# giech/usrp_nfc

Hardware: AMD Instinct MI355X
Metric: IQ Msamples/s -> decoded bits (2 Msps stream) (higher is better)
Workload: dtype f32 envelope / f64 window sums / u8 symbols; 1 GPU; configs[1]: Miller-only decode, synthetic IQ @2 Msps; input_kind=fc32 IQ, 8 B/sample (envelope computed in the kernel), samples_per_gpu=100000000, parallelism=time-chunk x1, edges_per_gpu=6627699, symbols_reader=3971547, symbols_tag=0, packets=101186, boundary_redos=0, exchange=none, stepping=sync, in_flight=1

## Files before the change

### usrp_nfc_amd/csrc/decode.hip.h

```cpp
#pragma once
#include <hip/hip_runtime.h>
#include <stdint.h>

#include "../../include/nfc_amd.h"
#include "scan.hip.h"

namespace nfc {

struct DecTables {
    const uint4 *mil_map;
    const uint2 *man_map;
    const uint16_t *mil_step;
    const uint16_t *man_step;
    int32_t nd;
    int32_t reader, tag;
    const uint2 *qmil_map;
    const uint16_t *qmil_step;
    uint32_t q_rep[2];
    uint32_t canon[4];
    int32_t q_ok;
};
__device__ __forceinline__ uint32_t byte_of(const uint32_t *w, uint32_t i) { return (w[i >> 2] >> (8u * (i & 3u))) & 0xFFu; }

struct DecCarry {
    int32_t mil_state, man_state;
    int32_t pkt_started[2];
    uint32_t pending[2];
};

constexpr int DEC_ITEMS = 16;
#ifndef NFC_DEC_GROUPS
#define NFC_DEC_GROUPS 2
#endif
constexpr int DEC_GROUPS = NFC_DEC_GROUPS;
constexpr int DEC_PER_THREAD = DEC_ITEMS * DEC_GROUPS;
constexpr int DEC_TILE = SCAN_BLOCK * DEC_PER_THREAD;
constexpr int DEC_LDS_ROWS = 512;
inline size_t dec_num_tiles(size_t n) { return (n + DEC_TILE - 1) / DEC_TILE; }

enum DecLdsUser { DEC_LDS_SPEC = 0, DEC_LDS_REDUCE = 1, DEC_LDS_APPLY = 2 };
inline size_t dec_table_bytes(DecLdsUser k, const DecTables &T) {
    const size_t rows = 4 * (size_t)T.nd, nr = T.reader ? 1 : 0, nt = T.tag ? 1 : 0;
    if (rows > (size_t)DEC_LDS_ROWS) return 0;
    switch (k) {
    case DEC_LDS_SPEC: return (nr + nt) * (rows * 16 + (rows + 1) * 8);
    case DEC_LDS_REDUCE: return nr * rows * 16 + nt * rows * 8;
    default: return nr * rows * 32 + nt * rows * 16;
    }
}

__device__ __forceinline__ void load_codes(const uint16_t *ecode, size_t base, size_t n, uint32_t (&c)[8]) {
    if (base + DEC_ITEMS <= n) {
        const uint4 a = *(const uint4 *)(ecode + base), b = *(const uint4 *)(ecode + base + 8);
        c[0] = a.x; c[1] = a.y; c[2] = a.z; c[3] = a.w;
        c[4] = b.x; c[5] = b.y; c[6] = b.z; c[7] = b.w;
    } else {
#pragma unroll
        for (int k = 0; k < 8; k++) {
            const size_t i = base + 2 * k;
            c[k] = (i < n ? (uint32_t)ecode[i] : 0u) | (i + 1 < n ? (uint32_t)ecode[i + 1] << 16 : 0u);
        }
    }
}
__device__ __forceinline__ void load_bytes16(const uint8_t *p, size_t base, size_t n, uint32_t fill, uint32_t (&w)[4]) {
    if (base + 16 <= n) {
        const uint4 a = *(const uint4 *)(p + base);
        w[0] = a.x; w[1] = a.y; w[2] = a.z; w[3] = a.w;
    } else {
#pragma unroll
        for (int k = 0; k < 4; k++) {
            uint32_t v = 0;
#pragma unroll
            for (int q = 0; q < 4; q++) {
                const size_t i = base + 4 * k + q;
                v |= (i < n ? (uint32_t)p[i] : fill) << (8 * q);
            }
            w[k] = v;
        }
    }
}

constexpr uint32_t PM_STOP = 0u, PM_START = 1u, PM_ID = 2u;
constexpr uint32_t FA_DB = 4u, FA_DC = 8u;
struct FrameAgg {
    uint32_t cnt[2];
    uint32_t nb[2], nc[2];
    uint32_t fl[2];
};
struct FrameAggOp {
    using T = FrameAgg;
    static __host__ __device__ __forceinline__ T identity() { return T{{0u, 0u}, {0u, 0u}, {0u, 0u}, {PM_ID, PM_ID}}; }
    static __device__ __forceinline__ T op(const T &a, const T &b) {
        T r;
#pragma unroll
        for (int t = 0; t < 2; t++) {
            const uint32_t ma = a.fl[t] & 3u, mb = b.fl[t] & 3u;
            const bool into_stopped = ma == PM_STOP;
            r.cnt[t] = a.cnt[t] + b.cnt[t];
            r.nb[t] = a.nb[t] + b.nb[t] - (into_stopped ? (b.fl[t] >> 2) & 1u : 0u);
            r.nc[t] = a.nc[t] + b.nc[t] - (into_stopped ? (b.fl[t] >> 3) & 1u : 0u);
            r.fl[t] = (mb == PM_ID ? ma : mb) | ((ma == PM_ID ? b.fl[t] : a.fl[t]) & (FA_DB | FA_DC));
        }
        return r;
// ... 242 lines not shown
            const uint32_t code = (c[g][k >> 1] >> (16 * (k & 1))) & 0xFFFFu;
            const uint32_t li = code & 0x3FFFu, route = code >> 14;
            uint32_t w = 0;
            if (route == 2u && T.reader) {
                const uint32_t e = mil[li * 16u + (st & 15u)];
                w = e >> 8;
                st = (st & ~15u) | (e & 15u);
            } else if (route == 1u && T.tag) {
                const uint32_t e = man[li * 8u + ((st >> 4) & 7u)];
                const uint32_t m = e >> 8;
                w = (m & 3u) ? ((m & 0xFCu) | 3u) : 0u;
                st = (st & 15u) | ((e & 15u) << 4);
            }
            ow[k >> 2] |= w << (8 * (k & 3));
        }
        const size_t gb = base + (size_t)DEC_ITEMS * g;
        if (gb < n) *(uint4 *)(outw + gb) = make_uint4(ow[0], ow[1], ow[2], ow[3]);
        mine = FramePkOp::op(mine, FramePkOp::pack(frame_agg_of(ow)));
    }
    TP_MARK();
    FramePk total_fa;
    *(uint4 *)(thread_aggs + tid) = make_uint4(mine.a[0], mine.a[1], mine.b[0], mine.b[1]);
    (void)block_exclusive<FramePkOp>(mine, lds2, total_fa);
    if (threadIdx.x == 0) frame_aggs[blockIdx.x] = FramePkOp::unpack(total_fa);
    TP_DONE(2);
}

constexpr int FW_WORDS = DEC_TILE * 2 / 32 + 4;
constexpr uint32_t ST_CLOSES = 512 * DEC_GROUPS;
struct TileStage {
    uint32_t *bits[2];
    uint32_t *close_bit[2];
    uint64_t *close_idx[2];
    uint32_t *drop_bit[2];
    FrameAgg *own;
    const uint32_t *epos;
    uint64_t g0;
    const uint64_t *idx64;
};
__device__ __forceinline__ void bitcopy_or(uint32_t *dst, uint32_t dst_bit, const uint32_t *src, uint32_t src_bit, uint32_t nbits, uint32_t cap_bits) {
    if (!nbits) return;
    const uint32_t w0 = dst_bit >> 5, nw = ((dst_bit & 31u) + nbits + 31u) >> 5, capw = (cap_bits + 31u) >> 5;
    for (uint32_t j = threadIdx.x; j < nw; j += blockDim.x) {
        if (w0 + j >= capw) break;
        const uint32_t lo = max(dst_bit, (w0 + j) << 5), hi = min(dst_bit + nbits, (w0 + j + 1u) << 5);
        const uint32_t sb = src_bit + (lo - dst_bit), k = sb & 31u;
        const uint32_t a = src[sb >> 5], b = k ? src[(sb >> 5) + 1u] : 0u;
        uint32_t v = (a >> k) | (k ? b << (32u - k) : 0u);
        const uint32_t cnt = hi - lo;
        if (cnt < 32u) v &= (1u << cnt) - 1u;
        v <<= (lo & 31u);
        if (v) atomicOr(dst + w0 + j, v);
    }
}

struct QMaps {
    uint32_t mil[2];
    uint32_t man[2];
};
struct ComposeQ {
    using T = QMaps;
    static __host__ __device__ __forceinline__ T identity() { return T{{0x03020100u, 0x07060504u}, {0x03020100u, 0x07060504u}}; }
    static __device__ __forceinline__ T op(const T &a, const T &b) {
        return T{{__builtin_amdgcn_perm(b.mil[1], b.mil[0], a.mil[0]), __builtin_amdgcn_perm(b.mil[1], b.mil[0], a.mil[1])},
                 {__builtin_amdgcn_perm(b.man[1], b.man[0], a.man[0]), __builtin_amdgcn_perm(b.man[1], b.man[0], a.man[1])}};
    }
    static __device__ __forceinline__ uint32_t step(const T &m, uint32_t st) {
        const uint32_t a = __builtin_amdgcn_perm(m.mil[1], m.mil[0], st & 7u) & 15u;
        const uint32_t b = __builtin_amdgcn_perm(m.man[1], m.man[0], (st >> 4) & 7u) & 15u;
        return a | (b << 4);
    }
};
struct DecSpec {
    QMaps map;
    uint32_t s_in;
    uint32_t needs;
    uint32_t pad[2];
};
static_assert(sizeof(DecSpec) == 32, "two 16-byte loads");
__device__ __forceinline__ bool map8_constant(const uint32_t (&m)[2]) { return m[0] == m[1] && m[0] == (m[0] & 0xFFu) * 0x01010101u; }
constexpr int DEC_RUNIN_MAX = 8;
static_assert(DEC_GROUPS >= 1 && DEC_GROUPS <= 2, "NFC_DEC_GROUPS: a thread's packed bits are accumulated in 64 bits (32 slots per group)");
static_assert(DEC_RUNIN_MAX * SCAN_BLOCK <= DEC_TILE, "the longest run-in fits inside the tile before");
template <bool LDS, int DECS>
__global__ __launch_bounds__(SCAN_BLOCK) void k_dec_spec(const uint16_t *ecode, size_t n, const uint32_t *n_dev, DecTables T, uint32_t state0, int runin_per_thread,
                                                        uint8_t *outw, FrameAgg *frame_aggs, DecSpec *spec, ZeroJob Z, TileStage S) {
    constexpr bool RD = (DECS & 1) != 0, TG = (DECS & 2) != 0;
    zero_words(Z);
    if (n_dev) n = min(n, (size_t)*n_dev);
    if ((size_t)blockIdx.x * DEC_TILE >= n) return;
    TP_DECL();
    extern __shared__ __attribute__((aligned(16))) unsigned char s_dec_tab[];
    const int trows = LDS ? 4 * T.nd : 0;
    uint16_t *const s_mil = (uint16_t *)s_dec_tab, *const s_man = s_mil + (RD ? trows * 8 : 0);
    uint2 *const s_milmap = (uint2 *)(s_man + (TG ? trows * 8 : 0)), *const s_manmap = s_milmap + (LDS && RD ? trows + 1 : 0);
    __shared__ QMaps lds[SCAN_WAVES];
    __shared__ FramePk lds2[SCAN_WAVES];
    __shared__ uint32_t s_needs;
    __shared__ uint32_t s_bits[2][FW_WORDS];
    __shared__ uint32_t s_drop[2];
    for (int i = threadIdx.x; i < 2 * FW_WORDS; i += SCAN_BLOCK) (&s_bits[0][0])[i] = 0u;
    if (threadIdx.x < 2) s_drop[threadIdx.x] = 0xFFFFFFFFu;
    const uint32_t ident = 4u * (uint32_t)T.nd;
    if (LDS) {
        const int rows = 4 * T.nd;
        for (int i = threadIdx.x; i <= rows; i += SCAN_BLOCK) {
            if (RD) s_milmap[i] = T.qmil_map[i];
            if (TG) s_manmap[i] = T.man_map[i];
        }
        for (int i = threadIdx.x; i < rows; i += SCAN_BLOCK) {
            if (RD) ((uint4 *)s_mil)[i] = ((const uint4 *)T.qmil_step)[i];
            if (TG) ((uint4 *)s_man)[i] = ((const uint4 *)T.man_step)[i];
        }
    }
    if (threadIdx.x == 0) s_needs = 0u;
    const size_t tid = (size_t)blockIdx.x * SCAN_BLOCK + threadIdx.x;
    const size_t base = tid * DEC_PER_THREAD;
    uint32_t c[DEC_GROUPS][8];
#pragma unroll
    for (int g = 0; g < DEC_GROUPS; g++) load_codes(ecode, base + DEC_ITEMS * g, n, c[g]);
    uint32_t rc[DEC_RUNIN_MAX / 2];
    const bool have_runin = blockIdx.x > 0;
    {
        const size_t r0 = (size_t)blockIdx.x * DEC_TILE - (size_t)runin_per_thread * SCAN_BLOCK + (size_t)threadIdx.x * runin_per_thread;
#pragma unroll
        for (int k = 0; k < DEC_RUNIN_MAX / 2; k++) rc[k] = (have_runin && 2 * k < runin_per_thread) ? *(const uint32_t *)(ecode + r0 + 2 * k) : 0u;
    }
    __syncthreads();
    TP_MARK();
    auto mil_row = [&](uint32_t code) __attribute__((always_inline)) -> uint2 {
        const uint32_t idx = (code >> 14) == 2u ? (code & 0x3FFFu) : ident;
        return LDS ? s_milmap[idx] : T.qmil_map[idx];
    };
    auto man_row = [&](uint32_t code) __attribute__((always_inline)) -> uint2 {
        const uint32_t idx = (code >> 14) == 1u ? (code & 0x3FFFu) : ident;
        return LDS ? s_manmap[idx] : T.man_map[idx];
    };
    auto then = [](const uint2 &a, const uint2 &b) __attribute__((always_inline)) -> uint2 {
        return make_uint2(__builtin_amdgcn_perm(b.y, b.x, a.x), __builtin_amdgcn_perm(b.y, b.x, a.y));
    };
    auto routes_of = [](uint32_t pair) __attribute__((always_inline)) -> uint32_t {
        const uint32_t r0 = (pair >> 14) & 3u, r1 = pair >> 30;
        return ((r0 == 2u || r1 == 2u) ? 1u : 0u) | ((r0 == 1u || r1 == 1u) ? 2u : 0u);
    };
    auto compose4 = [&](uint2 &am, uint2 &an, uint32_t w0, uint32_t w1) __attribute__((always_inline)) {
        const uint32_t c0 = w0 & 0xFFFFu, c1 = w0 >> 16, c2 = w1 & 0xFFFFu, c3 = w1 >> 16;
        if (RD) am = then(am, then(then(mil_row(c0), mil_row(c1)), then(mil_row(c2), mil_row(c3))));
        if (TG) an = then(an, then(then(man_row(c0), man_row(c1)), then(man_row(c2), man_row(c3))));
    };
    const QMaps idm = ComposeQ::identity();
    QMaps runin = idm;
    if (have_runin) {
        uint2 am = make_uint2(idm.mil[0], idm.mil[1]), an = make_uint2(idm.man[0], idm.man[1]);
#pragma unroll
        for (int k = 0; k < DEC_RUNIN_MAX / 2; k += 2)
            if (2 * k < runin_per_thread) compose4(am, an, rc[k], rc[k + 1]);
        const QMaps ra{{am.x, am.y}, {an.x, an.y}};
        (void)block_exclusive<ComposeQ>(ra, lds, runin);
    }
    uint32_t seen = 0u;
    uint2 am = make_uint2(idm.mil[0], idm.mil[1]), an = make_uint2(idm.man[0], idm.man[1]);
#ifndef NFC_DEC_CHAIN
#define NFC_DEC_CHAIN 8
#endif
    constexpr int CHAIN = NFC_DEC_CHAIN;
    static_assert(CHAIN == 16 || CHAIN == 8 || CHAIN == 4, "NFC_DEC_CHAIN");
    constexpr int NCH = DEC_PER_THREAD / CHAIN;
    uint2 pm[NCH], pn[NCH];
#pragma unroll
    for (int g = 0; g < DEC_GROUPS; g++) {
#pragma unroll
        for (int k = 0; k < 8; k += 2) {
            if (k % (CHAIN / 2) == 0) {
                pm[(16 * g + 2 * k) / CHAIN] = am;
                pn[(16 * g + 2 * k) / CHAIN] = an;
            }
            compose4(am, an, c[g][k], c[g][k + 1]);
            seen |= routes_of(c[g][k]) | routes_of(c[g][k + 1]);
        }
    }
    if (!RD) seen &= ~1u;
    if (!TG) seen &= ~2u;
    const QMaps agg{{am.x, am.y}, {an.x, an.y}};
    TP_MARK();
    QMaps total;
    const QMaps excl = block_exclusive<ComposeQ>(agg, lds, total);
    const QMaps upto = ComposeQ::op(runin, excl);
    const uint32_t dep = ((seen & 1u) && !map8_constant(upto.mil) ? 1u : 0u) | ((seen & 2u) && !map8_constant(upto.man) ? 2u : 0u);
    if (blockIdx.x > 0 && dep) atomicOr(&s_needs, dep);
    uint32_t st[NCH];
#pragma unroll
    for (int j = 0; j < NCH; j++) st[j] = ComposeQ::step(ComposeQ::op(upto, QMaps{{pm[j].x, pm[j].y}, {pn[j].x, pn[j].y}}), state0);
    TP_MARK();
    const uint16_t *mil = LDS ? s_mil : T.qmil_step;
    const uint16_t *man = LDS ? s_man : T.man_step;
    uint32_t ow[DEC_GROUPS][4];
#pragma unroll
    for (int g = 0; g < DEC_GROUPS; g++) ow[g][0] = ow[g][1] = ow[g][2] = ow[g][3] = 0u;
#pragma unroll
    for (int e = 0; e < CHAIN; e++) {
#pragma unroll
        for (int j = 0; j < NCH; j++) {
            const int g = (j * CHAIN) / DEC_ITEMS, k = (j * CHAIN) % DEC_ITEMS + e;
            const uint32_t code = (c[g][k >> 1] >> (16 * (k & 1))) & 0xFFFFu;
            const uint32_t li = code & 0x3FFFu, route = code >> 14;
            uint32_t w = 0;
            if (route == 2u && RD) {
                const uint32_t en = mil[li * 8u + (st[j] & 7u)];
                w = en >> 8;
                st[j] = (st[j] & ~15u) | (en & 15u);
            } else if (route == 1u && TG) {
                const uint32_t en = man[li * 8u + ((st[j] >> 4) & 7u)];
                const uint32_t m = en >> 8;
                w = (m & 3u) ? ((m & 0xFCu) | 3u) : 0u;
                st[j] = (st[j] & 15u) | ((en & 15u) << 4);
            }
            ow[g][k >> 2] |= w << (8 * (k & 3));
        }
    }
    FramePk mine = FramePkOp::identity();
#pragma unroll
    for (int g = 0; g < DEC_GROUPS; g++) {
        const size_t gb = base + (size_t)DEC_ITEMS * g;
        if (gb < n) *(uint4 *)(outw + gb) = make_uint4(ow[g][0], ow[g][1], ow[g][2], ow[g][3]);
        mine = FramePkOp::op(mine, FramePkOp::pack(frame_agg_of<DECS>(ow[g])));
    }
    TP_MARK();
    FramePk total_fa;
    const FramePk in_tile = block_exclusive<FramePkOp>(mine, lds2, total_fa);
    {
        FrameAgg before = FramePkOp::unpack(in_tile);
        uint64_t acc[2] = {0ull, 0ull};
        uint32_t cnt[2] = {0u, 0u};
        const uint32_t bo0[2] = {before.nb[0], before.nb[1]};
#pragma unroll
        for (int g = 0; g < DEC_GROUPS; g++) {
            if (ow[g][0] | ow[g][1] | ow[g][2] | ow[g][3]) {
                const SlotMasks m = slot_masks<DECS>(ow[g]);
                const uint32_t low = symbol_low_bits(ow[g]);
#pragma unroll
                for (int t = 0; t < 2; t++) {
                    if (!(t ? RD : TG) || !m.V[t]) continue;
                    const uint32_t started = pm_apply(before.fl[t], 1u);
                    const uint32_t bef = started_before(m, t, started);
                    const uint32_t appended = m.V[t] & ~m.ST[t] & (bef | ~m.SA[t]);
                    uint32_t cl = m.ST[t] & bef;
                    const uint32_t bo = bo0[t] + cnt[t];
                    const uint32_t nonid = m.ST[t] | m.SA[t];
                    if ((before.fl[t] & 3u) == PM_ID && nonid) {
                        const uint32_t first = nonid & (0u - nonid);
                        if (first & m.SA[t]) s_drop[t] = bo + (uint32_t)__popc(appended & (first - 1u));
                    }
                    acc[t] |= (uint64_t)compress32(low, appended) << cnt[t];
                    cnt[t] += (uint32_t)__popc(appended);
                    if (cl) {
                        const uint32_t co = before.nc[t], closes = cl;
                        while (cl) {
                            const uint32_t lowb = cl & (0u - cl);
                            const int k = (__ffs((int)cl) - 1) >> 1;
                            cl ^= lowb;
                            const uint32_t j = co + (uint32_t)__popc(closes & (lowb - 1u));
                            if (j < ST_CLOSES) {
                                const size_t e = base + (size_t)DEC_ITEMS * g + k;
                                S.close_bit[t][(size_t)blockIdx.x * ST_CLOSES + j] = bo + (uint32_t)__popc(appended & (lowb - 1u));
                                S.close_idx[t][(size_t)blockIdx.x * ST_CLOSES + j] = S.idx64 ? S.idx64[e] : S.g0 + (uint64_t)S.epos[e];
                            } else {
                                atomicOr(&s_needs, 4u);
                            }
                        }
                    }
                }
                if (g + 1 < DEC_GROUPS) before = FrameAggOp::op(before, frame_agg_of<DECS>(ow[g]));
            }
        }
#pragma unroll
        for (int t = 0; t < 2; t++) {
            if (!cnt[t]) continue;
            const uint32_t w = bo0[t] >> 5, sh = bo0[t] & 31u;
            const uint64_t lo = acc[t] << sh;
            const uint32_t hi = sh ? (uint32_t)(acc[t] >> (64u - sh)) : 0u;
            if (w + 2 < (uint32_t)FW_WORDS) {
                if ((uint32_t)lo) atomicOr(&s_bits[t][w], (uint32_t)lo);
                if ((uint32_t)(lo >> 32)) atomicOr(&s_bits[t][w + 1], (uint32_t)(lo >> 32));
                if (hi) atomicOr(&s_bits[t][w + 2], hi);
            }
        }
    }
    __syncthreads();
    const FrameAgg tile_fa = FramePkOp::unpack(total_fa);
#pragma unroll
    for (int t = 0; t < 2; t++) {
        if (!(t ? RD : TG)) continue;
        const uint32_t nw = min((uint32_t)FW_WORDS, (tile_fa.nb[t] + 31u) / 32u + 1u);
        for (uint32_t j = threadIdx.x; j < nw; j += SCAN_BLOCK) S.bits[t][(size_t)blockIdx.x * FW_WORDS + j] = s_bits[t][j];
    }
    if (threadIdx.x == 0) {
        frame_aggs[blockIdx.x] = tile_fa;
        S.own[blockIdx.x] = tile_fa;
        if (TG) S.drop_bit[0][blockIdx.x] = s_drop[0];
        if (RD) S.drop_bit[1][blockIdx.x] = s_drop[1];
// ... 439 lines not shown
```

### usrp_nfc_amd/csrc/decoder_tables.h

```cpp
#pragma once
#include <cmath>
#include <cstdint>
#include <vector>

namespace nfc {

enum : int { E_NONE = 0, E_TOO_SHORT = 2, E_TOO_LONG = 3, E_ENCODING = 4, E_INTERNAL = 5, E_WRONG_DUR = 6 };
constexpr double kFull = 9.44;
constexpr double kZero = 3.00;
constexpr double kHalf = kFull / 2;
constexpr double kZeroRem = kFull - kZero;
constexpr double kOneRem = kHalf - kZero;
constexpr double kOneHalf = kFull + kHalf;

enum : int { MS_BEGIN = 0, MS_ZS0 = 1, MS_OS0 = 2, MS_OS1 = 3 };
constexpr int kMillerStates = 16;
constexpr int kManchStates = 8;

struct Step {
    int next;
    int nout;
    int out[2];
};

// ... 141 lines not shown
                tm |= (uint32_t)(st.next & 15) << (4 * s);
                t.manch_out[((size_t)c * nd + d) * kManchStates + s] = pack_out(st);
            }
            t.manch_map[c * nd + d] = tm;
        }
    }
    return t;
}

struct MillerQuotient {
    bool ok = false;
    int classes = 0;
    uint8_t q_of[16], rep[8], canon[16];
    std::vector<uint64_t> map;
    std::vector<uint16_t> step;
};
inline MillerQuotient miller_quotient(const DecoderTables &t) {
    MillerQuotient q;
    const size_t rows = t.miller_map.size();
    int cls[16] = {0};
    for (;;) {
        int ncls[16], nid = 0;
        std::vector<std::vector<int>> sigs;
        for (int s = 0; s < 16; s++) {
            std::vector<int> sig{cls[s]};
            for (size_t r = 0; r < rows; r++) {
                sig.push_back(t.miller_out[r * 16 + s]);
                sig.push_back(cls[(t.miller_map[r] >> (4 * s)) & 15]);
            }
            int id = -1;
            for (int k = 0; k < nid; k++)
                if (sigs[k] == sig) id = k;
            if (id < 0) {
                id = nid++;
                sigs.push_back(sig);
            }
            ncls[s] = id;
        }
        bool same = true;
        for (int s = 0; s < 16; s++) same = same && ncls[s] == cls[s];
        for (int s = 0; s < 16; s++) cls[s] = ncls[s];
        if (same) break;
    }
    bool reach[16] = {false};
    reach[0] = true;
    for (bool grew = true; grew;) {
        grew = false;
        for (int s = 0; s < 16; s++)
            if (reach[s])
                for (size_t r = 0; r < rows; r++) {
                    const int nx = (int)((t.miller_map[r] >> (4 * s)) & 15);
                    if (!reach[nx]) reach[nx] = grew = true;
                }
    }
    int qid[16];
    for (int k = 0; k < 16; k++) qid[k] = -1;
    for (int s = 0; s < 16; s++)
        if (reach[s] && qid[cls[s]] < 0) {
            if (q.classes == 8) return q;
            q.rep[q.classes] = (uint8_t)s;
            qid[cls[s]] = q.classes++;
        }
    for (int s = 0; s < 16; s++) {
        q.q_of[s] = qid[cls[s]] >= 0 ? (uint8_t)qid[cls[s]] : (uint8_t)0xFF;
        q.canon[s] = qid[cls[s]] >= 0 ? q.rep[qid[cls[s]]] : (uint8_t)s;
    }
    for (int k = q.classes; k < 8; k++) q.rep[k] = q.rep[0];
    q.map.assign(rows, 0);
    q.step.assign(rows * 8, 0);
    for (size_t r = 0; r < rows; r++) {
        uint64_t m = 0;
        for (int k = 0; k < 8; k++) {
            const int s = q.rep[k < q.classes ? k : 0];
            const int nx = q.q_of[(t.miller_map[r] >> (4 * s)) & 15];
            m |= (uint64_t)nx << (8 * k);
            q.step[r * 8 + k] = (uint16_t)(nx | (t.miller_out[r * 16 + s] << 8));
        }
        q.map[r] = m;
    }
    q.ok = true;
    return q;
}

}
```

### usrp_nfc_amd/csrc/host_context.h

```cpp
#pragma once


namespace {

std::string g_create_error;

}

enum : int {
    TOT_RUNS = 0,
    TOT_EDGES = 8,
    TOT_DECMAP = 16,
    TOT_SPEC = 40,
    TOT_PKT0 = 72,
    TOT_PKT1 = 80,
    TOT_LAST2 = 88,
    TOT_NSYM = 96,
    TOT_CERT = 104,
    TOT_FRAME = 128,
    TOT_BYTES = 160
};

static_assert(sizeof(CertSummary) <= TOT_FRAME - TOT_CERT, "the verdict summary fits its slot of the totals");
struct DevState {
// ... 41 lines not shown
    if (const char *e = getenv("NFC_OWN_PREFIX_MAX")) s.own_prefix_max = strtoul(e, nullptr, 10);
    if (const char *e = getenv("NFC_WG_LONE")) {
        int a = 4, b = 64;
        if (sscanf(e, "%d,%d", &a, &b) >= 1) s.wg_lone = std::make_pair(a, b);
    }
    if (const char *e = getenv("NFC_WG_ROWBAL")) {
        std::array<double, 3> f{0.0, 1.0, 1.0};
        if (sscanf(e, "%lf,%lf,%lf", &f[0], &f[1], &f[2]) >= 2 && f[0] > 0.5 && f[0] < 1.5 && f[1] > 0.5 && f[1] < 1.5 && f[2] > 0.5 && f[2] < 1.5)
            s.rowbal_f = f;
        else s.wg_rowbal = atoi(e);
    }
    if (const char *e = getenv("NFC_RING")) {
        if (strcmp(e, "global") == 0) s.ring_global = true;
        else if (strcmp(e, "lds") == 0) s.ring_global = false;
    }
#endif
    return s;
}
}

struct nfc_ctx {
    nfc_params P;
    const KindKernels *kk = nullptr;
    int L, mx, Lpad, wpb, twords;
    double factor;
    double hi_plus, lo_a, lo_b, hi_a, hi_b;
    int bands_ok, fast_ok, nfold, wave_slots, lds_per_slot;
    int C_min;
    uint32_t ring_carried = 0;
    bool dec_spec = true, dec_spec_now = false;
    int dec_runin = 2, spec_off_left = 0, spec_fail_streak = 0;
    size_t dec_lds[3] = {0, 0, 0};
    bool bits_packed = false, sym_lazy = false, sym_own = false;
    FrameOut sym_P;
    uint32_t sym_n = 0, sym_tiles = 0;
    uint32_t decode_respeculated = 0;
    int lean = 1, lean_rounds = 0, lean_slots = 0;
    int n_cus = 1;
    double rowbal_f[5][3] = {{1, 1, 1}, {1, 1, 1}, {1.02, 1, 1}, {1.045, 1.004, 1}, {1.036, 1.015, 0.990}};
    bool rowbal_set = false;
    bool wg_rowbal = true;
    int wg = 1, wg_ok = 0, wg_nr = 4, wg_slots = 0, wg_slots_ahead = 0, wg_rounds = 0;
    int fine_left = 0, fine_adapt = 1, fine_mult = 4;
    size_t wg_lds = 0, wg_lds_base = 0, wg_lds_bulk_max = 0;
    bool wg_bulk = true;
    int wg_lone_max = 4, wg_lone_div = 64;
    int wg_rerun_lone = 1;
    int wg_ex_ok = 0, wg_ex_max = 0;
    size_t wg_ex_lds = 0;
    float lean_gfac = 1.3f, lean_gmin = 9.765625e-4f;
    int gring_ok = 0, gring_force = 0, wave_slots_g = 0;
    uint32_t own_prefix_max = OWN_PREFIX_MAX_TILES;
    int use_small = 1;
    double expect_ms = 0.3;
    bool spin_wait = true;
    uint64_t selmask;
    float eps;
    float i16_scale;
    size_t in_bytes_per_sample;
    hipStream_t st = nullptr;
    Stream own_st;
    Stream st_a;
    Event ev[8];
    DevBuf d_gring;
    bool state_dirty = false, dirty_fill_ring = false;
    float dirty_fill = 0.f;
    Carry dirty_carry;
    EdgeCarry dirty_ecarry;
    DecCarry dirty_dcarry;
    bool cert_pending = false;
    CertLaunch cert;
    bool fill_pending = false, fill_can_ride = false, fill_front = false;
    FillRider fill;
    uint32_t dbg_fill_rode = 0, dbg_fill_refront = 0;
    bool dbg_bad_launch = false, dbg_redo_submitted = false, dbg_no_submit_ahead = false, dbg_any = false, dbg_clk = false, dbg_trace = false;
    std::string dbg_clk_path;
    uint32_t batch_seq = 0;
    int timing = 0;
    Event kev[2 * 6];
    int n_kev = 0;
    std::string err;
    LaunchError launch_err;

    DevBuf d_mil_map, d_man_map, d_mil_out, d_man_out, d_qmil_map, d_qmil_step;
    uint8_t mil_q_of[16], mil_canon[16];
    DecTables T;

    DevBuf d_state, d_ring[NRING];
    PinBuf hs_pin{hipHostMallocMapped | hipHostMallocCoherent};
    DevState *hs = nullptr;
    void *hs_dev = nullptr;
    PinBuf h_stage;
    PinBuf h_pk_stage;
    PinBuf h_edge_stage;
    std::vector<uint64_t> edge_lut;
    PinBuf h_cflags;
    int ring_cur = 0;
    DevBuf d_neg_alt[NSUB - 1], d_pos_alt[NSUB - 1];
    uint32_t alt_free = (1u << (NSUB - 1)) - 1u;
    PinBuf hs_a[NSUB];
    Event ev_a[NSUB], ev_b[NSUB];
    Event kev_sub[NSUB][2];
    struct Submitted {
        const void *d_in = nullptr;
        uint32_t n = 0, seq = 0, nch = 0, chunk = 0;
        uint64_t g0 = 0;
        int slot = 0, planes = -1, ring_in = 0, timing = 0;
        uint32_t allocs = 0;
        bool fast = false, b_enqueued = false, timed = false, spec = false;
    } sub[NSUB];
    int sub_count = 0;
    uint32_t slot_next = 0;
    bool low_valid = false;
    size_t lean_lds_per_cu = 0;
    size_t ahead_lds_per_cu = 0;
    uint32_t stamp_b = 0;
    bool in_wait = false;
    uint32_t dbg_fast_waits = 0;
    uint32_t stats_redo_submitted = 0;
    Carry h_carry;
    EdgeCarry h_ecarry;
    DecCarry h_dcarry;
    uint64_t nseen = 0;

    DevBuf d_certinfo;
    DevBuf d_in, d_neg, d_pos, d_ringout[2], d_touched[2], d_info[2], d_ringin, d_meta, d_ver, d_cflags, d_list;
    DevBuf d_ecode, d_epos, d_eidx;
    bool edges_from_host = false;
    std::vector<nfc_edge> h_pushed;
    DevBuf d_states, d_sym[2], d_bits[2], d_pending[2][2], d_close_end[2],
        d_close_idx[2];
    DevBuf d_partials, d_partials2, d_aggs, d_faggs;
    DevBuf d_edge_rec;
    int edge_prefix = -1;
    DevBuf d_spec;
    DevBuf d_stage_bits[2], d_stage_cb[2], d_stage_ci[2], d_stage_q[2], d_stage_own;
    DevBuf d_pack;
    DevBuf d_gvtop;
    DevBuf d_seqout;
    uint32_t cap_edges = 0, cap_sym[2] = {0, 0};
    uint32_t alloc_edges = 0, alloc_sym[2] = {0, 0};
    uint64_t alloc_mark = 0;
    uint64_t cap_edges_floor = 0, cap_sym_floor[2] = {0, 0};
    double edge_rate = 0.125;
    double sym_rate[2] = {1.0, 2.0};
    int pend_cur = 0;
    RerunBook book;

    const void *last_in = nullptr;
    uint32_t last_n = 0, last_skip = 0;
    uint64_t last_g0 = 0;
    uint32_t n_edges = 0;
    uint32_t n_sym[2] = {0, 0}, n_close[2] = {0, 0}, n_bits[2] = {0, 0};
    bool have_outputs = false;
    nfc_stats stats;
    std::vector<nfc_packet> pk[2];
    bool pk_ready[2] = {false, false};
    DevBuf d_fr_rec[2], d_fr_bytes[2], d_fr_par[2], d_fr_tot;
    bool frames_ready = false;
    uint64_t fr_frames[2] = {0, 0}, fr_bytes[2] = {0, 0};
    Event fr_ev[2];
    float fr_ms = 0.f;
    bool fr_enqueued = false, fr_timed = false;
    frames::CtxArgs fr_args;
    struct Commands {
        bool on = false;
        bool batch = false;
// ... 157 lines not shown
```

### usrp_nfc_amd/csrc/nfc_amd.hip

```cpp
#include <hip/hip_runtime.h>
#include <hip/hip_ext.h>

#include <algorithm>
#include <atomic>
#include <chrono>
#include <cmath>
#include <cstdarg>
#include <cstdio>
#include <cstdlib>
#include <cstring>
#include <string>
#include <thread>
#include <array>
#include <functional>
#include <memory>
#include <optional>
#include <vector>

#include "../../include/nfc_amd.h"
#include "launch_check.h"
#include "decode.hip.h"
#include "decoder_tables.h"
#include "edges.hip.h"
#include "scan.hip.h"
// ... 182 lines not shown
    c->wg_slots_ahead = prop.multiProcessorCount * per_cu_ahead;
    if (c->wg_ok && c->wg && c->lean) c->ahead_lds_per_cu = c->wg_lds * (size_t)per_cu_ahead;
    c->wg_ex_lds = c->wg_lds_base + wg_stage_bytes(4, 2 * wg_flush_rounds(4));
    c->wg_ex_ok = c->wg_ok && c->mx <= 64 * 4 - 2 && c->L >= wg_round_samples(4) && c->wg_ex_lds <= 160 * 1024;
    if (c->wg_ex_ok) {
        const void *kx = (const void *)c->kk->wg_ex;
        if (c->wg_ex_lds > 64 * 1024) CRT(hipFuncSetAttribute(kx, hipFuncAttributeMaxDynamicSharedMemorySize, (int)c->wg_ex_lds));
        int fit = 0;
        CRT(hipOccupancyMaxActiveBlocksPerMultiprocessor(&fit, kx, 256, c->wg_ex_lds));
        if (fit < 1) c->wg_ex_ok = 0;
        c->wg_ex_max = prop.multiProcessorCount * std::max(1, std::min(4, fit));
    }
    if (sw.wg_ex) {
        if (*sw.wg_ex <= 0) c->wg_ex_ok = 0;
        else c->wg_ex_max = *sw.wg_ex;
    }
    if (!c->wg_rounds) c->wg_rounds = 8;
    if (sw.chunk_adapt) c->fine_adapt = *sw.chunk_adapt != 0;
    if (sw.chunk_mult) c->fine_mult = std::max(1, std::min(16, *sw.chunk_mult));
    if (sw.fill_front) c->fill_front = *sw.fill_front != 0;
    return NFC_OK;
}

int create_resources(nfc_ctx *c) {
    CRT(c->own_st.create());
    c->st = c->own_st;
    for (auto &e : c->ev) CRT(e.create());
    for (auto &e : c->kev) CRT(e.create());
    CRT(c->st_a.create());
    for (int b = 0; b < NSUB; b++) {
        CRT(c->ev_a[b].create(hipEventDisableTiming));
        CRT(c->ev_b[b].create(hipEventDisableTiming));
        CRT(c->kev_sub[b][0].create());
        CRT(c->kev_sub[b][1].create());
        CRT(c->hs_a[b].ensure(sizeof(DevState)));
        memset(c->hs_a[b].p, 0, sizeof(DevState));
    }
    const size_t lds = (size_t)c->wpb * c->Lpad * c->lds_per_slot;
    if (lds > 160 * 1024) return fail(nullptr, NFC_ERR_ARG, "av_window too large for one wave's LDS ring");
    if (lds > 64 * 1024) {
        for (int kind = 0; kind < N_KINDS; kind++)
            for (const ThrKernel kern : {kind_kernels(kind).thr[0], kind_kernels(kind).lean[0], kind_kernels(kind).lean[1]})
                CRT(hipFuncSetAttribute((const void *)kern, hipFuncAttributeMaxDynamicSharedMemorySize, (int)lds));
    }
    const nfc_params *p = &c->P;
    DecoderTables t = build_tables(p->samp_rate, c->mx);
    std::vector<uint8_t> milb(t.miller_map.size() * 16), manb(t.manch_map.size() * 8);
    for (size_t i = 0; i < t.miller_map.size(); i++)
        for (int s = 0; s < 16; s++) milb[i * 16 + s] = (uint8_t)((t.miller_map[i] >> (4 * s)) & 15u);
    for (size_t i = 0; i < t.manch_map.size(); i++)
        for (int s = 0; s < 8; s++) manb[i * 8 + s] = (uint8_t)((t.manch_map[i] >> (4 * s)) & 15u);
    std::vector<uint16_t> mils(milb.size()), mans(manb.size());
    for (size_t i = 0; i < milb.size(); i++) mils[i] = (uint16_t)(milb[i] | (t.miller_out[i] << 8));
    for (size_t i = 0; i < manb.size(); i++) mans[i] = (uint16_t)(manb[i] | (t.manch_out[i] << 8));
    for (int s = 0; s < 16; s++) milb.push_back((uint8_t)s);
    for (int s = 0; s < 8; s++) manb.push_back((uint8_t)s);
    CRT(c->d_mil_map.ensure(milb.size()));
    CRT(c->d_man_map.ensure(manb.size()));
    CRT(c->d_mil_out.ensure(mils.size() * 2));
    CRT(c->d_man_out.ensure(mans.size() * 2));
    CRT(hipMemcpy(c->d_mil_map.p, milb.data(), milb.size(), hipMemcpyHostToDevice));
    CRT(hipMemcpy(c->d_man_map.p, manb.data(), manb.size(), hipMemcpyHostToDevice));
    CRT(hipMemcpy(c->d_mil_out.p, mils.data(), mils.size() * 2, hipMemcpyHostToDevice));
    CRT(hipMemcpy(c->d_man_out.p, mans.data(), mans.size() * 2, hipMemcpyHostToDevice));
    {
        const MillerQuotient q = miller_quotient(t);
        c->T.q_ok = q.ok ? 1 : 0;
        for (int k = 0; k < 16; k++) c->mil_q_of[k] = q.ok ? q.q_of[k] : (uint8_t)0xFF;
        uint8_t canon[16], rep[8] = {0};
        for (int k = 0; k < 16; k++) canon[k] = q.ok ? q.canon[k] : (uint8_t)k;
        if (q.ok) memcpy(rep, q.rep, 8);
        memcpy(c->T.canon, canon, 16);
        memcpy(c->T.q_rep, rep, 8);
        memcpy(c->mil_canon, canon, 16);
        if (q.ok) {
            std::vector<uint64_t> qm(q.map);
            qm.push_back(0x0706050403020100ull);
            CRT(c->d_qmil_map.ensure(qm.size() * 8));
            CRT(c->d_qmil_step.ensure(q.step.size() * 2 + 16));
            CRT(hipMemcpy(c->d_qmil_map.p, qm.data(), qm.size() * 8, hipMemcpyHostToDevice));
            CRT(hipMemcpy(c->d_qmil_step.p, q.step.data(), q.step.size() * 2, hipMemcpyHostToDevice));
            c->T.qmil_map = c->d_qmil_map.as<uint2>();
            c->T.qmil_step = c->d_qmil_step.as<uint16_t>();
        }
    }
    c->T.mil_map = c->d_mil_map.as<uint4>();
    c->T.man_map = c->d_man_map.as<uint2>();
    c->T.mil_step = c->d_mil_out.as<uint16_t>();
    c->T.man_step = c->d_man_out.as<uint16_t>();
    c->T.nd = c->mx + 1;
    c->T.reader = p->enable_reader ? 1 : 0;
    c->T.tag = p->enable_tag ? 1 : 0;
    for (int k = 0; k < 3; k++) c->dec_lds[k] = dec_table_bytes((DecLdsUser)k, c->T);
    CRT(c->d_state.ensure(sizeof(DevState)));
    CRT(c->hs_pin.ensure(sizeof(DevState)));
    c->hs = c->hs_pin.as<DevState>();
    memset(c->hs, 0, sizeof(DevState));
    CRT(hipHostGetDevicePointer(&c->hs_dev, c->hs, 0));
    for (int b = 0; b < NRING; b++) {
        CRT(c->d_ring[b].ensure((size_t)c->Lpad * 4));
        CRT(hipMemset(c->d_ring[b].p, 0, (size_t)c->Lpad * 4));
    }
    for (int b = 0; b < 2; b++) {
        CRT(c->d_pending[b][0].ensure(1024));
        CRT(c->d_pending[b][1].ensure(1024));
    }
    push_state(c, 1);
    CRT(hipStreamSynchronize(c->st));
    return NFC_OK;
}
#undef CRT
}

extern "C" {

int nfc_abi_version(void) { return NFC_AMD_ABI_VERSION; }

int nfc_plan_row_cut(uint32_t n, uint32_t C, uint32_t rs, uint32_t cus, uint32_t rows, const double *factors, uint32_t max_len, uint32_t out[10]) {
    if (!out || !rs || !C || !cus || (rows >= 2 && !factors)) return NFC_ERR_ARG;
    const RowCut t = (rows >= 2 && rows <= 4) ? plan_row_cut(n, C, rs, cus, rows, factors, max_len) : equal_cut(n, C, cus);
    for (int r = 0; r < 4; r++) {
        out[r] = t.row_len[r];
        out[4 + r] = t.row_start[r];
    }
    out[8] = t.row_div;
    out[9] = t.nch;
    return t.by_row ? 1 : 0;
}

int nfc_device_count(void) {
    int n = 0;
    if (hipGetDeviceCount(&n) != hipSuccess) return 0;
    return n;
}

const char *nfc_last_error(const nfc_ctx *ctx) { return ctx ? ctx->err.c_str() : g_create_error.c_str(); }
extern "C++" {
namespace nfc { void note_call_error(const char *text) { g_create_error = text; } }
}

int nfc_create(const nfc_params *p, nfc_ctx **out) {
    if (!p || !out) return fail(nullptr, NFC_ERR_ARG, "null argument");
    *out = nullptr;
    float scale_arg = 0.f;
    if (int rc = create_check_args(p, &scale_arg)) return rc;
    const Switches sw = read_switches();
    std::unique_ptr<nfc_ctx, void (*)(nfc_ctx *)> c(new nfc_ctx(), nfc_destroy);
    if (int rc = create_plan_params(c.get(), p, sw, scale_arg)) return rc;
    if (int rc = create_plan_device(c.get(), sw)) return rc;
    if (int rc = create_resources(c.get())) return rc;
    *out = c.release();
    return NFC_OK;
}

void nfc_destroy(nfc_ctx *c) {
    if (!c) return;
    (void)hipSetDevice(c->P.device);
    if (c->st_a) (void)hipStreamSynchronize(c->st_a);
    if (c->st && c->st == c->own_st) (void)hipStreamSynchronize(c->st);
    else (void)hipDeviceSynchronize();
    delete c;
}

int nfc_push_device(nfc_ctx *c, const void *dev_samples, size_t n) {
    LaunchScope launch_scope_(c ? &c->launch_err : nullptr);
    if (!c) return NFC_ERR_ARG;
// ... 1102 lines not shown
```

Before: 450,800 Msamples/s.

## Precompute LDS walk tables and packed row addresses in speculative decode

Adds host-built 'walk' tables that store the XOR-delta of the next state and the final output byte, so the per-symbol decode loop becomes an LDS u16 load at a precomputed address plus an XOR, with no branching on route. Row addresses for the map and walk tables are computed two symbols at a time with packed 16-bit min/shift/add, steering non-routed codes to an identity or zero row. The route 'seen' check is derived from the minimum row address, and output bytes are merged with v_perm. The aim is to cut ALU and branch work in the LDS path of the decode kernel. The cost is more live registers for the precomputed row pairs and reliance on the LDS address layout fitting in 16 bits.

```diff
diff --git a/usrp_nfc_amd/csrc/decode.hip.h b/usrp_nfc_amd/csrc/decode.hip.h
--- a/usrp_nfc_amd/csrc/decode.hip.h
+++ b/usrp_nfc_amd/csrc/decode.hip.h
@@ -19,6 +19,7 @@
     uint32_t q_rep[2];
     uint32_t canon[4];
     int32_t q_ok;
+    const uint16_t *qmil_walk, *man_walk;
 };
 __device__ __forceinline__ uint32_t byte_of(const uint32_t *w, uint32_t i) { return (w[i >> 2] >> (8u * (i & 3u))) & 0xFFu; }
 
@@ -427,6 +428,33 @@
 constexpr int DEC_RUNIN_MAX = 8;
 static_assert(DEC_GROUPS >= 1 && DEC_GROUPS <= 2, "NFC_DEC_GROUPS: a thread's packed bits are accumulated in 64 bits (32 slots per group)");
 static_assert(DEC_RUNIN_MAX * SCAN_BLOCK <= DEC_TILE, "the longest run-in fits inside the tile before");
+typedef unsigned short dec_u16x2 __attribute__((ext_vector_type(2)));
+typedef uint32_t dec_u32x2 __attribute__((ext_vector_type(2)));
+typedef __attribute__((address_space(3))) const unsigned char *dec_lds_ptr;
+__device__ __forceinline__ uint32_t lds_addr(const void *p) { return (uint32_t)(uintptr_t)(dec_lds_ptr)p; }
+__device__ __forceinline__ uint32_t twice16(uint32_t v) { return (v & 0xFFFFu) | (v << 16); }
+struct RowTable {
+    uint32_t route, walk, walk_other, map, map_other;
+};
+__device__ __forceinline__ RowTable row_table(uint32_t route, const void *walk, const void *map, uint32_t ident, const void *zero) {
+    return RowTable{twice16(route << 14), twice16(lds_addr(walk)), twice16(((lds_addr(zero) - lds_addr(walk)) & 0xFFFFu) >> 4), twice16(lds_addr(map)), twice16(ident)};
+}
+struct RowPair {
+    uint32_t walk, map;
+};
+__device__ __forceinline__ dec_u16x2 u16x2(uint32_t v) { return __builtin_bit_cast(dec_u16x2, v); }
+__device__ __forceinline__ RowPair row_pair(uint32_t codes, const RowTable &t) {
+    const dec_u16x2 x = u16x2(codes ^ t.route);
+    const dec_u16x2 w = __builtin_elementwise_min(x, u16x2(t.walk_other)), m = __builtin_elementwise_min(x, u16x2(t.map_other));
+    return RowPair{__builtin_bit_cast(uint32_t, (dec_u16x2)((w << (dec_u16x2)(4)) + u16x2(t.walk))), __builtin_bit_cast(uint32_t, (dec_u16x2)((m << (dec_u16x2)(3)) + u16x2(t.map)))};
+}
+__device__ __forceinline__ uint32_t half16(uint32_t pair, int hi) { return hi ? pair >> 16 : pair & 0xFFFFu; }
+__device__ __forceinline__ uint32_t half16_plus(uint32_t pair, int hi, uint32_t v) {
+    uint32_t r;
+    if (hi) asm("v_add_u32_sdwa %0, %1, %2 dst_sel:DWORD dst_unused:UNUSED_PAD src0_sel:WORD_1 src1_sel:DWORD" : "=v"(r) : "v"(pair), "v"(v));
+    else asm("v_add_u32_sdwa %0, %1, %2 dst_sel:DWORD dst_unused:UNUSED_PAD src0_sel:WORD_0 src1_sel:DWORD" : "=v"(r) : "v"(pair), "v"(v));
+    return r;
+}
 template <bool LDS, int DECS>
 __global__ __launch_bounds__(SCAN_BLOCK) void k_dec_spec(const uint16_t *ecode, size_t n, const uint32_t *n_dev, DecTables T, uint32_t state0, int runin_per_thread,
                                                         uint8_t *outw, FrameAgg *frame_aggs, DecSpec *spec, ZeroJob Z, TileStage S) {
@@ -444,8 +472,10 @@
     __shared__ uint32_t s_needs;
     __shared__ uint32_t s_bits[2][FW_WORDS];
     __shared__ uint32_t s_drop[2];
+    __shared__ __attribute__((aligned(16))) uint32_t s_dec_zero[4];
     for (int i = threadIdx.x; i < 2 * FW_WORDS; i += SCAN_BLOCK) (&s_bits[0][0])[i] = 0u;
     if (threadIdx.x < 2) s_drop[threadIdx.x] = 0xFFFFFFFFu;
+    if (threadIdx.x < 4) s_dec_zero[threadIdx.x] = 0u;
     const uint32_t ident = 4u * (uint32_t)T.nd;
     if (LDS) {
         const int rows = 4 * T.nd;
@@ -454,8 +484,8 @@
             if (TG) s_manmap[i] = T.man_map[i];
         }
         for (int i = threadIdx.x; i < rows; i += SCAN_BLOCK) {
-            if (RD) ((uint4 *)s_mil)[i] = ((const uint4 *)T.qmil_step)[i];
-            if (TG) ((uint4 *)s_man)[i] = ((const uint4 *)T.man_step)[i];
+            if (RD) ((uint4 *)s_mil)[i] = ((const uint4 *)T.qmil_walk)[i];
+            if (TG) ((uint4 *)s_man)[i] = ((const uint4 *)T.man_walk)[i];
         }
     }
     if (threadIdx.x == 0) s_needs = 0u;
@@ -473,13 +503,21 @@
     }
     __syncthreads();
     TP_MARK();
-    auto mil_row = [&](uint32_t code) __attribute__((always_inline)) -> uint2 {
-        const uint32_t idx = (code >> 14) == 2u ? (code & 0x3FFFu) : ident;
-        return LDS ? s_milmap[idx] : T.qmil_map[idx];
+    const RowTable tab_m = row_table(2u, s_mil, s_milmap, ident, s_dec_zero), tab_n = row_table(1u, s_man, s_manmap, ident, s_dec_zero);
+    auto rows_m = [&](uint32_t codes) __attribute__((always_inline)) { return row_pair(codes, tab_m); };
+    auto rows_n = [&](uint32_t codes) __attribute__((always_inline)) { return row_pair(codes, tab_n); };
+    auto lds_u16 = [](uint32_t addr) __attribute__((always_inline)) -> uint32_t { return *(__attribute__((address_space(3))) const uint16_t *)(dec_lds_ptr)(uintptr_t)addr; };
+    auto lds_u2 = [](uint32_t addr) __attribute__((always_inline)) -> uint2 {
+        const dec_u32x2 v = *(__attribute__((address_space(3))) const dec_u32x2 *)(dec_lds_ptr)(uintptr_t)addr;
+        return make_uint2(v.x, v.y);
     };
-    auto man_row = [&](uint32_t code) __attribute__((always_inline)) -> uint2 {
-        const uint32_t idx = (code >> 14) == 1u ? (code & 0x3FFFu) : ident;
-        return LDS ? s_manmap[idx] : T.man_map[idx];
+    auto mil_row = [&](uint32_t h) __attribute__((always_inline)) -> uint2 {
+        if (LDS) return lds_u2(h);
+        return T.qmil_map[(h >> 14) == 2u ? (h & 0x3FFFu) : ident];
+    };
+    auto man_row = [&](uint32_t h) __attribute__((always_inline)) -> uint2 {
+        if (LDS) return lds_u2(h);
+        return T.man_map[(h >> 14) == 1u ? (h & 0x3FFFu) : ident];
     };
     auto then = [](const uint2 &a, const uint2 &b) __attribute__((always_inline)) -> uint2 {
         return make_uint2(__builtin_amdgcn_perm(b.y, b.x, a.x), __builtin_amdgcn_perm(b.y, b.x, a.y));
@@ -488,10 +526,13 @@
         const uint32_t r0 = (pair >> 14) & 3u, r1 = pair >> 30;
         return ((r0 == 2u || r1 == 2u) ? 1u : 0u) | ((r0 == 1u || r1 == 1u) ? 2u : 0u);
     };
-    auto compose4 = [&](uint2 &am, uint2 &an, uint32_t w0, uint32_t w1) __attribute__((always_inline)) {
-        const uint32_t c0 = w0 & 0xFFFFu, c1 = w0 >> 16, c2 = w1 & 0xFFFFu, c3 = w1 >> 16;
-        if (RD) am = then(am, then(then(mil_row(c0), mil_row(c1)), then(mil_row(c2), mil_row(c3))));
-        if (TG) an = then(an, then(then(man_row(c0), man_row(c1)), then(man_row(c2), man_row(c3))));
+    auto compose4 = [&](uint2 &am, uint2 &an, uint32_t m0, uint32_t m1, uint32_t n0, uint32_t n1) __attribute__((always_inline)) {
+        if (RD) am = then(am, then(then(mil_row(half16(m0, 0)), mil_row(half16(m0, 1))), then(mil_row(half16(m1, 0)), mil_row(half16(m1, 1)))));
+        if (TG) an = then(an, then(then(man_row(half16(n0, 0)), man_row(half16(n0, 1))), then(man_row(half16(n1, 0)), man_row(half16(n1, 1)))));
+    };
+    auto compose4_codes = [&](uint2 &am, uint2 &an, uint32_t w0, uint32_t w1) __attribute__((always_inline)) {
+        if (LDS) compose4(am, an, RD ? rows_m(w0).map : 0u, RD ? rows_m(w1).map : 0u, TG ? rows_n(w0).map : 0u, TG ? rows_n(w1).map : 0u);
+        else compose4(am, an, w0, w1, w0, w1);
     };
     const QMaps idm = ComposeQ::identity();
     QMaps runin = idm;
@@ -499,7 +540,7 @@
         uint2 am = make_uint2(idm.mil[0], idm.mil[1]), an = make_uint2(idm.man[0], idm.man[1]);
 #pragma unroll
         for (int k = 0; k < DEC_RUNIN_MAX / 2; k += 2)
-            if (2 * k < runin_per_thread) compose4(am, an, rc[k], rc[k + 1]);
+            if (2 * k < runin_per_thread) compose4_codes(am, an, rc[k], rc[k + 1]);
         const QMaps ra{{am.x, am.y}, {an.x, an.y}};
         (void)block_exclusive<ComposeQ>(ra, lds, runin);
     }
@@ -512,6 +553,20 @@
     static_assert(CHAIN == 16 || CHAIN == 8 || CHAIN == 4, "NFC_DEC_CHAIN");
     constexpr int NCH = DEC_PER_THREAD / CHAIN;
     uint2 pm[NCH], pn[NCH];
+    RowPair rm[DEC_GROUPS][8], rn[DEC_GROUPS][8];
+    if (LDS) {
+        dec_u16x2 low_m = u16x2(tab_m.map_other), low_n = u16x2(tab_n.map_other);
+#pragma unroll
+        for (int g = 0; g < DEC_GROUPS; g++) {
+#pragma unroll
+            for (int k = 0; k < 8; k++) {
+                if (RD) low_m = __builtin_elementwise_min(low_m, u16x2((rm[g][k] = rows_m(c[g][k])).map));
+                if (TG) low_n = __builtin_elementwise_min(low_n, u16x2((rn[g][k] = rows_n(c[g][k])).map));
+            }
+        }
+        const uint32_t id_m = (tab_m.map & 0xFFFFu) + 8u * ident, id_n = (tab_n.map & 0xFFFFu) + 8u * ident;
+        seen = (RD && min((uint32_t)low_m.x, (uint32_t)low_m.y) < id_m ? 1u : 0u) | (TG && min((uint32_t)low_n.x, (uint32_t)low_n.y) < id_n ? 2u : 0u);
+    }
 #pragma unroll
     for (int g = 0; g < DEC_GROUPS; g++) {
 #pragma unroll
@@ -520,8 +575,12 @@
                 pm[(16 * g + 2 * k) / CHAIN] = am;
                 pn[(16 * g + 2 * k) / CHAIN] = an;
             }
-            compose4(am, an, c[g][k], c[g][k + 1]);
-            seen |= routes_of(c[g][k]) | routes_of(c[g][k + 1]);
+            if (LDS) {
+                compose4(am, an, RD ? rm[g][k].map : 0u, RD ? rm[g][k + 1].map : 0u, TG ? rn[g][k].map : 0u, TG ? rn[g][k + 1].map : 0u);
+            } else {
+                compose4(am, an, c[g][k], c[g][k + 1], c[g][k], c[g][k + 1]);
+                seen |= routes_of(c[g][k]) | routes_of(c[g][k + 1]);
+            }
         }
     }
     if (!RD) seen &= ~1u;
@@ -537,30 +596,57 @@
 #pragma unroll
     for (int j = 0; j < NCH; j++) st[j] = ComposeQ::step(ComposeQ::op(upto, QMaps{{pm[j].x, pm[j].y}, {pn[j].x, pn[j].y}}), state0);
     TP_MARK();
-    const uint16_t *mil = LDS ? s_mil : T.qmil_step;
-    const uint16_t *man = LDS ? s_man : T.man_step;
     uint32_t ow[DEC_GROUPS][4];
 #pragma unroll
     for (int g = 0; g < DEC_GROUPS; g++) ow[g][0] = ow[g][1] = ow[g][2] = ow[g][3] = 0u;
-#pragma unroll
-    for (int e = 0; e < CHAIN; e++) {
+    if constexpr (LDS) {
+        uint32_t sm[NCH], sn[NCH];
 #pragma unroll
         for (int j = 0; j < NCH; j++) {
-            const int g = (j * CHAIN) / DEC_ITEMS, k = (j * CHAIN) % DEC_ITEMS + e;
-            const uint32_t code = (c[g][k >> 1] >> (16 * (k & 1))) & 0xFFFFu;
-            const uint32_t li = code & 0x3FFFu, route = code >> 14;
-            uint32_t w = 0;
-            if (route == 2u && RD) {
-                const uint32_t en = mil[li * 8u + (st[j] & 7u)];
-                w = en >> 8;
-                st[j] = (st[j] & ~15u) | (en & 15u);
-            } else if (route == 1u && TG) {
-                const uint32_t en = man[li * 8u + ((st[j] >> 4) & 7u)];
-                const uint32_t m = en >> 8;
-                w = (m & 3u) ? ((m & 0xFCu) | 3u) : 0u;
-                st[j] = (st[j] & 15u) | ((en & 15u) << 4);
-            }
-            ow[g][k >> 2] |= w << (8 * (k & 3));
+            sm[j] = (st[j] & 7u) << 1;
+            sn[j] = (st[j] >> 3) & 14u;
+        }
+#pragma unroll
+        for (int e = 0; e < CHAIN; e++) {
+#pragma unroll
+            for (int j = 0; j < NCH; j++) {
+                const int g = (j * CHAIN) / DEC_ITEMS, k = (j * CHAIN) % DEC_ITEMS + e;
+                uint32_t x = 0u;
+                if (RD) {
+                    const uint32_t en = lds_u16(half16_plus(rm[g][k >> 1].walk, k & 1, sm[j]));
+                    sm[j] ^= en & 0xFFu;
+                    x = en;
+                }
+                if (TG) {
+                    const uint32_t en = lds_u16(half16_plus(rn[g][k >> 1].walk, k & 1, sn[j]));
+                    sn[j] ^= en & 0xFFu;
+                    x |= en;
+                }
+                ow[g][k >> 2] = __builtin_amdgcn_perm(x, ow[g][k >> 2], 0x03020100u ^ (0x05u ^ (uint32_t)(k & 3)) << (8 * (k & 3)));
+            }
+        }
+    } else {
+        const uint16_t *mil = T.qmil_step, *man = T.man_step;
+#pragma unroll
+        for (int e = 0; e < CHAIN; e++) {
+#pragma unroll
+            for (int j = 0; j < NCH; j++) {
+                const int g = (j * CHAIN) / DEC_ITEMS, k = (j * CHAIN) % DEC_ITEMS + e;
+                const uint32_t code = (c[g][k >> 1] >> (16 * (k & 1))) & 0xFFFFu;
+                const uint32_t li = code & 0x3FFFu, route = code >> 14;
+                uint32_t w = 0;
+                if (route == 2u && RD) {
+                    const uint32_t en = mil[li * 8u + (st[j] & 7u)];
+                    w = en >> 8;
+                    st[j] = (st[j] & ~15u) | (en & 15u);
+                } else if (route == 1u && TG) {
+                    const uint32_t en = man[li * 8u + ((st[j] >> 4) & 7u)];
+                    const uint32_t m = en >> 8;
+                    w = (m & 3u) ? ((m & 0xFCu) | 3u) : 0u;
+                    st[j] = (st[j] & 15u) | ((en & 15u) << 4);
+                }
+                ow[g][k >> 2] |= w << (8 * (k & 3));
+            }
         }
     }
     FramePk mine = FramePkOp::identity();
diff --git a/usrp_nfc_amd/csrc/decoder_tables.h b/usrp_nfc_amd/csrc/decoder_tables.h
--- a/usrp_nfc_amd/csrc/decoder_tables.h
+++ b/usrp_nfc_amd/csrc/decoder_tables.h
@@ -247,4 +247,14 @@
     return q;
 }
 
-}
+inline std::vector<uint16_t> spec_walk_rows(const std::vector<uint16_t> &step, bool manchester) {
+    std::vector<uint16_t> w(step.size());
+    for (size_t i = 0; i < step.size(); i++) {
+        const uint32_t k = (uint32_t)(i & 7), next = step[i] & 7u, m = step[i] >> 8;
+        const uint32_t out = manchester ? ((m & 3u) ? ((m & 0xFCu) | 3u) : 0u) : m;
+        w[i] = (uint16_t)(((next ^ k) << 1) | (out << 8));
+    }
+    return w;
+}
+
+}
diff --git a/usrp_nfc_amd/csrc/host_context.h b/usrp_nfc_amd/csrc/host_context.h
--- a/usrp_nfc_amd/csrc/host_context.h
+++ b/usrp_nfc_amd/csrc/host_context.h
@@ -147,7 +147,7 @@
     std::string err;
     LaunchError launch_err;
 
-    DevBuf d_mil_map, d_man_map, d_mil_out, d_man_out, d_qmil_map, d_qmil_step;
+    DevBuf d_mil_map, d_man_map, d_mil_out, d_man_out, d_qmil_map, d_qmil_step, d_qmil_walk, d_man_walk;
     uint8_t mil_q_of[16], mil_canon[16];
     DecTables T;
 
diff --git a/usrp_nfc_amd/csrc/nfc_amd.hip b/usrp_nfc_amd/csrc/nfc_amd.hip
--- a/usrp_nfc_amd/csrc/nfc_amd.hip
+++ b/usrp_nfc_amd/csrc/nfc_amd.hip
@@ -288,6 +288,13 @@
             CRT(hipMemcpy(c->d_qmil_step.p, q.step.data(), q.step.size() * 2, hipMemcpyHostToDevice));
             c->T.qmil_map = c->d_qmil_map.as<uint2>();
             c->T.qmil_step = c->d_qmil_step.as<uint16_t>();
+            const std::vector<uint16_t> qw = spec_walk_rows(q.step, false), nw = spec_walk_rows(mans, true);
+            CRT(c->d_qmil_walk.ensure(qw.size() * 2));
+            CRT(c->d_man_walk.ensure(nw.size() * 2));
+            CRT(hipMemcpy(c->d_qmil_walk.p, qw.data(), qw.size() * 2, hipMemcpyHostToDevice));
+            CRT(hipMemcpy(c->d_man_walk.p, nw.data(), nw.size() * 2, hipMemcpyHostToDevice));
+            c->T.qmil_walk = c->d_qmil_walk.as<uint16_t>();
+            c->T.man_walk = c->d_man_walk.as<uint16_t>();
         }
     }
     c->T.mil_map = c->d_mil_map.as<uint4>();
```

Result: no change. 457,900 Msamples/s, median of 3 (+1.6%).
